# SAP/nested-hashing-psi

Hardware: AMD Instinct MI355X
Metric: server PIE ciphertexts/sec (higher is better)
Workload: dtype u64

## Files before the change

### nested_hashing_psi_amd/csrc/kernels_pie.hip

```cpp
#include <stdlib.h>

#include <cassert>

#include <algorithm>

#include "kernels.hpp"
#include "madasm.h"
#include "stage_a_common.h"
#include "pie_arith.h"

namespace piehip {

static const u32 TPB = 256;

typedef u64 u64x2 __attribute__((ext_vector_type(2)));


template <int BPT>
__global__ void __launch_bounds__(TPB) stage_a_kernel(const DevConsts *__restrict__ dc, u32 N, u32 L, u32 K, u32 b, u32 E,
                                                      const u64 *__restrict__ idx, const u64 *__restrict__ minus,
                                                      const u64 *__restrict__ db, u64 *__restrict__ acc, u32 bstride, u32 h0,
                                                      u32 nq, u32 q)
{
    const u32 n = 2 * (blockIdx.x * TPB + threadIdx.x);
// ... 686 lines not shown
        const Mod qk = ld_mod(c, k);
        u64 col[Lp];
#pragma unroll
        for (u32 j = 0; j < Lp; j++) col[j] = c->tQF_modq[j][k];
        const u64 tp = c->tPinv_modq[k], nq = neg_u(qk.q);
#pragma unroll
        for (int p = 0; p < NP; p++) {
            if (MAD && L <= 6) {
                ColAcc a = {itot[p].lo, 0, 0};
#pragma unroll
                for (u32 j = 0; j < Lp; j++) colacc_mac(a, split30(yp[p][j]), split30(col[j]));
                if (PONLY)
                    ;
                else if (PRE)
                    a.c0 += d[p][k];
                else
                    colacc_mac(a, split30(d[p][k]), split30(tp));
                out[p][k] = (L <= 5 && lz) ? colacc_reduce123_lazy(a, qk, nq) : colacc_reduce<(L > 5)>(a, qk, nq);
            } else {
                U128 acc = dot128<Lp, MAD>(yp[p], col);
                if (PONLY)
                    ;
                else if (PRE)
                    add128(acc, U128{d[p][k], 0});
                else
                    mac128(acc, d[p][k], tp);
                add128(acc, itot[p]);
                out[p][k] = reduce128(acc, qk);
            }
        }
    }
}

template <bool FOLD, u32 L, bool MAD, bool PONLY>
__device__ __forceinline__ void scale_round_comp(const DevConsts *__restrict__ dc, u32 N, u32 n, const u64 *__restrict__ pin,
                                                 u64 *__restrict__ pout, bool fold_out, bool lz)
{
    const u32 H = N / 2;
    constexpr u32 M = 2 * L + 1;
    constexpr int NP = FOLD ? 2 : 1;
    u64 x[NP][M], y[NP][L];
#pragma unroll
    for (u32 a = PONLY ? L : 0; a < M; a++) {
        if (FOLD) {
            PIE_ITER_FENCE();
            const DcC c = dc_iter(dc);
            const u32 ak = a < L ? a : 0, aj = a < L ? 0 : a - L;
            const u64 q = c->mod[a].q, nq = neg_u(q), u = pin[(size_t)a * N], v = pin[(size_t)a * N + H];
            const u64 wa = a < L ? c->fold_iat[ak] : c->fold_iap[aj], was = a < L ? c->fold_iat_sh[ak] : c->fold_iap_sh[aj];
            const u64 wb = a < L ? c->fold_ibt[ak] : c->fold_ibp[aj], wbs = a < L ? c->fold_ibt_sh[ak] : c->fold_ibp_sh[aj];
            x[0][a] = shoup63(u + v, wa, was, nq);
            x[NP - 1][a] = shoup63(u + (4 * q - v), wb, wbs, nq);
        } else {
            x[0][a] = pin[(size_t)a * N];
        }
    }
    scale_round_core<L, MAD, NP, FOLD, PONLY>(dc, x, y, lz);
#pragma unroll
    for (u32 k = 0; k < L; k++) {
        PIE_ITER_FENCE();
        if (FOLD) {
            u64 y0 = y[0][k], y1 = y[NP - 1][k];
            if (fold_out) fold_store(dc, k, y[0][k], y[NP - 1][k], y0, y1);
            pout[(size_t)k * N] = y0;
            pout[(size_t)k * N + H] = y1;
        } else {
            pout[(size_t)k * N] = y[0][k];
        }
    }
}
template <bool FOLD, u32 L, bool MAD, bool P01 = false, bool P2 = false>
__global__ void __launch_bounds__(TPB) scale_round_kernel(const DevConsts *__restrict__ dc, u32 N, const u64 *__restrict__ d,
                                                          u64 *__restrict__ out01, size_t stride01,
                                                          u64 *__restrict__ out2, size_t stride2, u32 fold_comp2)
{
    const u32 n = blockIdx.x * TPB + threadIdx.x;
    if (n >= (FOLD ? N / 2 : N)) return;
    const u32 comp = blockIdx.y, bin = blockIdx.z;
    constexpr u32 M = 2 * L + 1;
    const u64 *pin = d + ((size_t)(bin * 3 + comp) * M) * N + n;
    u64 *pout = comp < 2 ? out01 + (size_t)bin * stride01 + (size_t)comp * L * N + n : out2 + (size_t)bin * stride2 + n;
    const bool lz = FOLD && MAD && comp < 2 && !fold_comp2;
    if (P01 && comp < 2)
        scale_round_comp<FOLD, L, MAD, true>(dc, N, n, pin, pout, true, lz);
    else if (P2 && comp == 2)
        scale_round_comp<FOLD, L, MAD, true>(dc, N, n, pin, pout, fold_comp2, lz);
    else
        scale_round_comp<FOLD, L, MAD, false>(dc, N, n, pin, pout, comp < 2 || fold_comp2, lz);
}
void launch_scale_round(const DevConsts *dc, u32 N, u32 L, const u64 *d, u32 nb, u64 *out01, size_t stride01, u64 *out2,
                        size_t stride2, hipStream_t st, bool small_moduli, bool fold, bool fold_comp2, bool p_only01, bool p_only2)
{
    assert(!p_only01 || (small_moduli && fold_comp2 == p_only2));
    assert(!p_only2 || p_only01);
    dim3 grid(((fold ? N / 2 : N) + TPB - 1) / TPB, 3, nb);
#define SRK2(F_, L_) \
    hipLaunchKernelGGL((scale_round_kernel<F_, L_, true, true, true>), grid, dim3(TPB), 0, st, dc, N, d, out01, stride01, out2, stride2, F_ ? 1u : 0u)
#define SRK(F_, L_, M_, P_) \
    hipLaunchKernelGGL((scale_round_kernel<F_, L_, M_, P_>), grid, dim3(TPB), 0, st, dc, N, d, out01, stride01, out2, stride2, (fold_comp2 && F_) ? 1u : 0u)
#define SRL(L_)                                                                        \
    case L_:                                                                           \
        if (p_only2) {                                                                 \
            if (fold) SRK2(true, L_); else SRK2(false, L_);                            \
        } else if (p_only01) {                                                                \
            if (fold) SRK(true, L_, true, true); else SRK(false, L_, true, true);      \
        } else if (small_moduli) {                                                     \
            if (fold) SRK(true, L_, true, false); else SRK(false, L_, true, false);    \
        } else {                                                                       \
            if (fold) SRK(true, L_, false, false); else SRK(false, L_, false, false);  \
        }                                                                              \
        break;
    switch (L) { SRL(1) SRL(2) SRL(3) SRL(4) SRL(5) SRL(6) SRL(7) }
#undef SRK
#undef SRK2
#undef SRL
}

__device__ __forceinline__ u64 digit_lift(const DevConsts *dc, u32 i, u32 j, u64 v)
{
    const Mod &mj = dc->mod[j];
    const u64 qi = dc->mod[i].q;
    u64 r = (qi < 2 * mj.q) ? (v >= mj.q ? v - mj.q : v) : barrett128(0, v, mj);
    if (v > qi / 2) r = submod(r, dc->qi_modqj[i][j], mj.q);
    return r;
}
template <bool FOLD>
__global__ void __launch_bounds__(TPB) digits_kernel(const DevConsts *__restrict__ dc, u32 N, u32 L, const u64 *__restrict__ d2,
                                                     size_t stride2, u64 *__restrict__ dig)
{
    const u32 n = blockIdx.x * TPB + threadIdx.x;
    const u32 H = N / 2;
    if (n >= (FOLD ? H : N)) return;
    const u32 i = blockIdx.y / L, j = blockIdx.y % L, bin = blockIdx.z;
    const u64 *pin = d2 + (size_t)bin * stride2 + (size_t)i * N + n;
    u64 *pout = dig + (((size_t)bin * L + i) * L + j) * N + n;
    if (FOLD) {
        u64 y0, y1;
        fold_store(dc, j, digit_lift(dc, i, j, pin[0]), digit_lift(dc, i, j, pin[H]), y0, y1);
        pout[0] = y0;
        pout[H] = y1;
    } else {
        pout[0] = digit_lift(dc, i, j, pin[0]);
    }
}
void launch_digits(const DevConsts *dc, u32 N, u32 L, const u64 *d2, size_t stride2, u32 nb, u64 *dig, hipStream_t st, bool fold)
{
    dim3 grid(((fold ? N / 2 : N) + TPB - 1) / TPB, L * L, nb);
    if (fold)
        hipLaunchKernelGGL(digits_kernel<true>, grid, dim3(TPB), 0, st, dc, N, L, d2, stride2, dig);
    else
        hipLaunchKernelGGL(digits_kernel<false>, grid, dim3(TPB), 0, st, dc, N, L, d2, stride2, dig);
}

template <bool MAD, int KP, int RPT = 1, bool EQ = false>
__global__ void __launch_bounds__(TPB) relin_mac_kernel(const DevConsts *__restrict__ dc, u32 N, u32 L, const u64 *__restrict__ d01,
                                                        size_t stride01, const u64 *__restrict__ dig,
                                                        const u64 *__restrict__ key0, const u64 *__restrict__ mask,
                                                        u64 *__restrict__ out, const u32 *__restrict__ out_map,
                                                        size_t key_stride, u32 key_group, u32 T, u32 mask_div, u32 nb,
                                                        const u64 *__restrict__ eqp, u32 eqp_M)
{
    static_assert(RPT == 1 || MAD, "two rows per thread: the column-accumulator path");
    static_assert(!EQ || MAD, "the own-limb term: the column-accumulator path");
    constexpr bool TILE = KP > 0;
    constexpr u32 TT = TILE ? TPB / (KP ? KP : 1) : 1;
    __shared__ u64x2 s_tile[TILE ? 2 * RPT : 1][TILE ? TPB : 1];
    u32 n = 2 * (blockIdx.x * TPB + threadIdx.x);
    u32 std_pair = 0;
    if (TILE) {
        const u32 tiles = T / TT, slice = blockIdx.x / tiles, tau0 = (blockIdx.x % tiles) * TT;
        const u32 k = threadIdx.x / TT, tt = threadIdx.x % TT;
        n = 2 * (slice * KP * T + k * T + tau0 + tt);
        std_pair = slice * KP * T + KP * tau0;
    }
    if (n >= N) return;
    const u32 j = blockIdx.y;
    u32 rows[RPT];
    bool has[RPT];
    if (RPT == 1) {
        rows[0] = blockIdx.z, has[0] = true;
    } else {
        const u32 k = blockIdx.z / key_group, q = blockIdx.z % key_group;
        rows[0] = 2 * k * key_group + q, has[0] = rows[0] < nb;
        rows[RPT - 1] = rows[0] + key_group, has[RPT - 1] = rows[RPT - 1] < nb;
        if (!has[0]) return;
    }
    const u32 bin = rows[0];
    const u64 *key = key0 + (size_t)(bin % key_group) * key_stride;
    const Mod m = dc->mod[j];
    const size_t LN = (size_t)L * N;
    const u32 po = TILE ? 0 : (out_map ? out_map[n] : n);
    u64x2 res[RPT][2];
    if (MAD) {
        ColAcc a[RPT][2][2];
#pragma unroll
        for (int r = 0; r < RPT; r++)
#pragma unroll
            for (int c = 0; c < 2; c++) a[r][c][0] = a[r][c][1] = ColAcc{0, 0, 0};
        for (u32 i = 0; i < L; i++) {
            const u64x2 k0 = *reinterpret_cast<const u64x2 *>(key + (((size_t)i * 2 + 0) * L + j) * N + n);
            const u64x2 k1 = *reinterpret_cast<const u64x2 *>(key + (((size_t)i * 2 + 1) * L + j) * N + n);
            const Split30 k0x = split30(k0.x), k0y = split30(k0.y), k1x = split30(k1.x), k1y = split30(k1.y);
#pragma unroll
            for (int r = 0; r < RPT; r++) {
                if (r && !has[r]) continue;
                const u64x2 d = *reinterpret_cast<const u64x2 *>(dig + (((size_t)rows[r] * L + i) * L + j) * N + n);
                const Split30 dx = split30(d.x), dy = split30(d.y);
                colacc_mac(a[r][0][0], dx, k0x);
                colacc_mac(a[r][0][1], dy, k0y);
                colacc_mac(a[r][1][0], dx, k1x);
                colacc_mac(a[r][1][1], dy, k1y);
            }
        }
        const u64 nq = 0 - m.q;
        if (EQ) {
            const u64 n2q = neg_u(2 * m.q), n4q = neg_u(4 * m.q);
            const u64 tp = dc->tPinv_modq[j], tpsh = dc->tPinv_modq_sh[j];
            const size_t MN = (size_t)eqp_M * N;
#pragma unroll
            for (int r = 0; r < RPT; r++) {
                if (r && !has[r]) continue;
                const u64 *pe = eqp + (size_t)rows[r] * 4 * MN + (size_t)j * N + n;
                const u64x2 va0 = *reinterpret_cast<const u64x2 *>(pe), va1 = *reinterpret_cast<const u64x2 *>(pe + MN),
                            vb0 = *reinterpret_cast<const u64x2 *>(pe + 2 * MN), vb1 = *reinterpret_cast<const u64x2 *>(pe + 3 * MN);
#pragma unroll
                for (int k = 0; k < 2; k++) {
                    const Split30 sa0 = split30(csub_u(csub_u(k ? va0.y : va0.x, n4q), n2q)), sa1 = split30(csub_u(csub_u(k ? va1.y : va1.x, n4q), n2q));
                    const Split30 sb0 = split30(csub_u(csub_u(k ? vb0.y : vb0.x, n4q), n2q)), sb1 = split30(csub_u(csub_u(k ? vb1.y : vb1.x, n4q), n2q));
                    ColAcc t = {0, 0, 0};
                    colacc_mac(t, sa0, sb0);
                    const u64 v0 = shoup63_lazy(colacc_reduce123_lazy(t, m, nq), tp, tpsh, nq);
                    t = ColAcc{0, 0, 0};
                    colacc_mac(t, sa0, sb1);
                    colacc_mac(t, sa1, sb0);
                    const u64 v1 = shoup63_lazy(colacc_reduce123_lazy(t, m, nq), tp, tpsh, nq);
                    a[r][0][k].c0 += v0 & 0x3FFFFFFFull, a[r][0][k].c1 += v0 >> 30;
                    a[r][1][k].c0 += v1 & 0x3FFFFFFFull, a[r][1][k].c1 += v1 >> 30;
                }
            }
        }
#pragma unroll
        for (int r = 0; r < RPT; r++) {
            if (r && !has[r]) continue;
            u64x2 mk;
            if (mask) mk = *reinterpret_cast<const u64x2 *>(mask + (size_t)(rows[r] / mask_div) * LN + (size_t)j * N + n);
#pragma unroll
            for (int c = 0; c < 2; c++) {
                const u64x2 s = *reinterpret_cast<const u64x2 *>(d01 + (size_t)rows[r] * stride01 + (size_t)c * LN + (size_t)j * N + n);
                a[r][c][0].c0 += s.x;
                a[r][c][1].c0 += s.y;
                res[r][c].x = colacc_reduce<false>(a[r][c][0], m, nq);
                res[r][c].y = colacc_reduce<false>(a[r][c][1], m, nq);
                if (mask) {
                    ColAcc p0 = {0, 0, 0}, p1 = {0, 0, 0};
                    colacc_mac(p0, split30(res[r][c].x), split30(mk.x));
                    colacc_mac(p1, split30(res[r][c].y), split30(mk.y));
                    res[r][c].x = colacc_reduce<false>(p0, m, nq);
                    res[r][c].y = colacc_reduce<false>(p1, m, nq);
                }
            }
        }
    } else {
        u64x2 mk;
        if (mask) mk = *reinterpret_cast<const u64x2 *>(mask + (size_t)(bin / mask_div) * LN + (size_t)j * N + n);
        U128 acc[2][2];
#pragma unroll
        for (int c = 0; c < 2; c++)
#pragma unroll
            for (int e = 0; e < 2; e++) acc[c][e] = U128{0, 0};
        for (u32 i = 0; i < L; i++) {
            const u64x2 d = *reinterpret_cast<const u64x2 *>(dig + (((size_t)bin * L + i) * L + j) * N + n);
            const u64x2 k0 = *reinterpret_cast<const u64x2 *>(key + (((size_t)i * 2 + 0) * L + j) * N + n);
            const u64x2 k1 = *reinterpret_cast<const u64x2 *>(key + (((size_t)i * 2 + 1) * L + j) * N + n);
            mac128(acc[0][0], d.x, k0.x);
            mac128(acc[0][1], d.y, k0.y);
            mac128(acc[1][0], d.x, k1.x);
            mac128(acc[1][1], d.y, k1.y);
        }
#pragma unroll
        for (int c = 0; c < 2; c++) {
            const u64x2 s = *reinterpret_cast<const u64x2 *>(d01 + (size_t)bin * stride01 + (size_t)c * LN + (size_t)j * N + n);
            add128(acc[c][0], U128{s.x, 0});
            add128(acc[c][1], U128{s.y, 0});
            res[0][c].x = reduce128(acc[c][0], m);
            res[0][c].y = reduce128(acc[c][1], m);
            if (mask) {
                res[0][c].x = mulmod(res[0][c].x, mk.x, m);
                res[0][c].y = mulmod(res[0][c].y, mk.y, m);
            }
        }
    }
#pragma unroll
    for (int r = 0; r < RPT; r++)
#pragma unroll
        for (int c = 0; c < 2; c++) {
            if (r && !has[r]) continue;
            const u64x2 v = res[r][c];
            if (TILE)
                s_tile[2 * r + c][KP * (threadIdx.x % TT) + threadIdx.x / TT] = v;
            else
                *reinterpret_cast<u64x2 *>(out + ((size_t)rows[r] * 2 + c) * LN + (size_t)j * N + po) = v;
        }
    if (TILE) {
        __syncthreads();
#pragma unroll
        for (int r = 0; r < RPT; r++)
#pragma unroll
            for (int c = 0; c < 2; c++) {
                if (r && !has[r]) continue;
                *reinterpret_cast<u64x2 *>(out + ((size_t)rows[r] * 2 + c) * LN + (size_t)j * N + 2 * (std_pair + threadIdx.x)) = s_tile[2 * r + c][threadIdx.x];
            }
    }
}
void launch_relin_mac(const DevConsts *dc, u32 N, u32 L, const u64 *d01, size_t stride01, const u64 *dig, const u64 *key,
                      const u64 *mask, u64 *out, u32 nb, hipStream_t st, bool small_moduli, const u32 *out_map, size_t key_stride,
                      u32 key_group, u32 sigma_T, u32 sigma_kp, u32 mask_div, const u64 *eqp, u32 eqp_M)
{
    assert(!eqp || (small_moduli && eqp_M >= L));
    if (!key_group) key_group = 1;
    if (!mask_div) mask_div = 1;
    const bool tile = out_map && (sigma_kp == 16 || sigma_kp == 8) && sigma_T >= TPB / sigma_kp && sigma_T % (TPB / sigma_kp) == 0 &&
                      (N / 2) % TPB == 0;
    const int kp = tile ? (int)sigma_kp : 0;
    const bool two = small_moduli && nb >= 2 * key_group;
    const u32 zrows = two ? ((nb + 2 * key_group - 1) / (2 * key_group)) * key_group : nb;
    dim3 grid((N / 2 + TPB - 1) / TPB, L, zrows);
#define RME(M_, K_, R_, E_)                                                                                                            \
    hipLaunchKernelGGL((relin_mac_kernel<M_, K_, R_, E_>), grid, dim3(TPB), 0, st, dc, N, L, d01, stride01, dig, key, mask, out, out_map, \
                       key_stride, key_group, sigma_T, mask_div, nb, eqp, eqp_M)
#define RM(M_, K_, R_) RME(M_, K_, R_, false)
#define RQ(K_, R_) RME(true, K_, R_, true)
    if (eqp && two) {
        if (kp == 16) RQ(16, 2); else if (kp == 8) RQ(8, 2); else RQ(0, 2);
    } else if (eqp) {
        if (kp == 16) RQ(16, 1); else if (kp == 8) RQ(8, 1); else RQ(0, 1);
    } else if (two) {
        if (kp == 16) RM(true, 16, 2); else if (kp == 8) RM(true, 8, 2); else RM(true, 0, 2);
    } else if (small_moduli) {
        if (kp == 16) RM(true, 16, 1); else if (kp == 8) RM(true, 8, 1); else RM(true, 0, 1);
    } else {
        if (kp == 16) RM(false, 16, 1); else if (kp == 8) RM(false, 8, 1); else RM(false, 0, 1);
    }
#undef RQ
#undef RM
#undef RME
}

template <int KP>
__global__ void __launch_bounds__(TPB) deg2_finish_kernel(const DevConsts *__restrict__ dc, u32 N, u32 L, const u64 *__restrict__ d,
                                                          const u64 *__restrict__ eqp, u32 eqp_M, const u64 *__restrict__ mask,
                                                          u64 *__restrict__ out, u32 T, u32 mask_div)
{
    constexpr u32 TT = TPB / KP;
    __shared__ u64x2 s_tile[3][TPB];
    const u32 tiles = T / TT, slice = blockIdx.x / tiles, tau0 = (blockIdx.x % tiles) * TT;
    const u32 kk = threadIdx.x / TT, tt = threadIdx.x % TT;
    const u32 n = 2 * (slice * KP * T + kk * T + tau0 + tt);
    const u32 std_pair = slice * KP * T + KP * tau0;
    const u32 j = blockIdx.y, row = blockIdx.z;
    const Mod m = dc->mod[j];
    const size_t LN = (size_t)L * N, MN = (size_t)eqp_M * N;
    const u64 nq = 0 - m.q, n2q = neg_u(2 * m.q), n4q = neg_u(4 * m.q);
    const u64 tp = dc->tPinv_modq[j], tpsh = dc->tPinv_modq_sh[j];
    const u64 *pe = eqp + (size_t)row * 4 * MN + (size_t)j * N + n;
    const u64x2 va0 = *reinterpret_cast<const u64x2 *>(pe), va1 = *reinterpret_cast<const u64x2 *>(pe + MN),
                vb0 = *reinterpret_cast<const u64x2 *>(pe + 2 * MN), vb1 = *reinterpret_cast<const u64x2 *>(pe + 3 * MN);
    const u64x2 mk = *reinterpret_cast<const u64x2 *>(mask + (size_t)(row / mask_div) * LN + (size_t)j * N + n);
    u64x2 s[3];
#pragma unroll
    for (int c = 0; c < 3; c++) s[c] = *reinterpret_cast<const u64x2 *>(d + ((size_t)row * 3 + c) * LN + (size_t)j * N + n);
    u64 res[3][2];
#pragma unroll
    for (int k = 0; k < 2; k++) {
        const Split30 sa0 = split30(csub_u(csub_u(k ? va0.y : va0.x, n4q), n2q)), sa1 = split30(csub_u(csub_u(k ? va1.y : va1.x, n4q), n2q));
        const Split30 sb0 = split30(csub_u(csub_u(k ? vb0.y : vb0.x, n4q), n2q)), sb1 = split30(csub_u(csub_u(k ? vb1.y : vb1.x, n4q), n2q));
        const Split30 smk = split30(k ? mk.y : mk.x);
        u64 v[3];
        ColAcc t = {0, 0, 0};
        colacc_mac(t, sa0, sb0);
        v[0] = shoup63_lazy(colacc_reduce123_lazy(t, m, nq), tp, tpsh, nq);
        t = ColAcc{0, 0, 0};
        colacc_mac(t, sa0, sb1);
        colacc_mac(t, sa1, sb0);
        v[1] = shoup63_lazy(colacc_reduce123_lazy(t, m, nq), tp, tpsh, nq);
        t = ColAcc{0, 0, 0};
        colacc_mac(t, sa1, sb1);
        v[2] = shoup63_lazy(colacc_reduce123_lazy(t, m, nq), tp, tpsh, nq);
#pragma unroll
        for (int c = 0; c < 3; c++) {
            ColAcc a = {(k ? s[c].y : s[c].x) + (v[c] & 0x3FFFFFFFull), v[c] >> 30, 0};
            ColAcc p = {0, 0, 0};
            colacc_mac(p, split30(colacc_reduce<false>(a, m, nq)), smk);
            res[c][k] = colacc_reduce<false>(p, m, nq);
        }
    }
#pragma unroll
    for (int c = 0; c < 3; c++) s_tile[c][KP * tt + kk] = u64x2{res[c][0], res[c][1]};
    __syncthreads();
#pragma unroll
    for (int c = 0; c < 3; c++)
        *reinterpret_cast<u64x2 *>(out + ((size_t)row * 3 + c) * LN + (size_t)j * N + 2 * (std_pair + threadIdx.x)) = s_tile[c][threadIdx.x];
}
bool deg2_finish_applies(u32 N, u32 sigma_T, u32 sigma_kp)
{
    return sigma_kp == 8 && sigma_T >= TPB / sigma_kp && sigma_T % (TPB / sigma_kp) == 0 && (N / 2) % TPB == 0;
}
void launch_deg2_finish(const DevConsts *dc, u32 N, u32 L, const u64 *d, const u64 *eqp, u32 eqp_M, const u64 *mask, u64 *out, u32 nb,
                        hipStream_t st, u32 sigma_T, u32 sigma_kp, u32 mask_div)
{
    assert(deg2_finish_applies(N, sigma_T, sigma_kp) && eqp_M >= L);
    dim3 grid(N / 2 / TPB, L, nb);
    hipLaunchKernelGGL(deg2_finish_kernel<8>, grid, dim3(TPB), 0, st, dc, N, L, d, eqp, eqp_M, mask, out, sigma_T, mask_div ? mask_div : 1);
}

__global__ void host_flag_kernel(volatile u64 *flag, u64 value)
{
    *flag = value;
    __threadfence_system();
}
void launch_host_flag(u64 *flag_dev, u64 value, hipStream_t st)
{
    hipLaunchKernelGGL(host_flag_kernel, dim3(1), dim3(1), 0, st, (volatile u64 *)flag_dev, value);
}

__global__ void __launch_bounds__(TPB) ct_add_kernel(const DevConsts *dc, u32 N, u32 L, const u64 *__restrict__ x,
                                                     const u64 *__restrict__ y, u64 *__restrict__ out)
{
    const u32 n = blockIdx.x * TPB + threadIdx.x;
    if (n >= N) return;
    const u32 l = blockIdx.y % L;
    const size_t o = ((size_t)blockIdx.z * 2 * L + blockIdx.y) * N + n;
    out[o] = addmod(x[o], y[o], dc->mod[l].q);
}
void launch_ct_add(const DevConsts *dc, u32 N, u32 L, const u64 *x, const u64 *y, u64 *out, u32 nct, hipStream_t st)
{
    dim3 grid((N + TPB - 1) / TPB, 2 * L, nct);
    hipLaunchKernelGGL(ct_add_kernel, grid, dim3(TPB), 0, st, dc, N, L, x, y, out);
}
__global__ void __launch_bounds__(TPB) ct_mul_plain_kernel(const DevConsts *dc, u32 N, u32 L, const u64 *__restrict__ x,
                                                           const u64 *__restrict__ pt, size_t pt_stride,
                                                           u64 *__restrict__ out, u32 pt_div)
{
    const u32 n = blockIdx.x * TPB + threadIdx.x;
    if (n >= N) return;
    const u32 l = blockIdx.y % L;
    const size_t o = ((size_t)blockIdx.z * 2 * L + blockIdx.y) * N + n;
    out[o] = mulmod(x[o], pt[(size_t)(blockIdx.z / pt_div) * pt_stride + (size_t)l * N + n], dc->mod[l]);
}
__global__ void __launch_bounds__(TPB) ctn_mul_plain_kernel(const DevConsts *dc, u32 N, u32 L, const u64 *__restrict__ x,
                                                            const u64 *__restrict__ pt, size_t pt_stride,
                                                            u64 *__restrict__ out, u32 pt_div, u32 comps)
{
    const u32 n = blockIdx.x * TPB + threadIdx.x;
    if (n >= N) return;
    const u32 l = blockIdx.y % L;
    const size_t o = ((size_t)blockIdx.z * comps * L + blockIdx.y) * N + n;
    out[o] = mulmod(x[o], pt[(size_t)(blockIdx.z / pt_div) * pt_stride + (size_t)l * N + n], dc->mod[l]);
}
void launch_ct_mul_plain(const DevConsts *dc, u32 N, u32 L, const u64 *x, const u64 *pt, size_t pt_stride, u64 *out,
                         u32 nct, hipStream_t st, u32 pt_div, u32 comps)
{
    dim3 grid((N + TPB - 1) / TPB, comps * L, nct);
    if (comps == 2)
        hipLaunchKernelGGL(ct_mul_plain_kernel, grid, dim3(TPB), 0, st, dc, N, L, x, pt, pt_stride, out, pt_div ? pt_div : 1);
    else
        hipLaunchKernelGGL(ctn_mul_plain_kernel, grid, dim3(TPB), 0, st, dc, N, L, x, pt, pt_stride, out, pt_div ? pt_div : 1, comps);
}

template <int L, int KEEP>
__global__ void __launch_bounds__(TPB) limb_drop_kernel(const DevConsts *__restrict__ dc, u32 N, u32 blocks_per_poly,
                                                        const u64 *__restrict__ in, u64 *__restrict__ out)
{
    const u32 poly = blockIdx.x / blocks_per_poly;
    const u32 n = (blockIdx.x % blocks_per_poly) * TPB + threadIdx.x;
    if (n >= N) return;
    const u64 *pin = in + (size_t)poly * L * N + n;
    u64 c[L];
#pragma unroll
    for (int i = 0; i < L; i++) c[i] = pin[(size_t)i * N];
#pragma unroll
    for (int l = L - 1; l >= KEEP; l--) {
        const u64 ql = dc->mod[l].q;
        const u64 v = c[l];
        const u64 s = (u64)((int64_t)((ql >> 1) - v) >> 63);
#pragma unroll
        for (int i = 0; i < l; i++) {
            const u64 off = dc->drop_off[l][i];
            const u64 x = c[i] - v + off + (s & (ql - off));
            c[i] = mul_shoup_u(x, dc->drop_inv[l][i], dc->drop_inv_sh[l][i], dc->mod[i].q, dc->drop_negq[i]);
        }
    }
    u64 *pout = out + (size_t)poly * KEEP * N + n;
#pragma unroll
    for (int i = 0; i < KEEP; i++) pout[(size_t)i * N] = c[i];
}
bool launch_limb_drop(const DevConsts *dc, u32 N, u32 L, u32 keep, const u64 *in, u64 *out, u32 npoly, hipStream_t st)
{
    if (keep < 1 || keep >= L || L > MAX_L || !npoly) return false;
    const u32 bpp = (N + TPB - 1) / TPB;
    const dim3 grid(bpp * npoly), block(TPB);
#define DROP_(L_, K_)                                                                                          \
    case (L_) * 8 + (K_):                                                                                      \
        hipLaunchKernelGGL((limb_drop_kernel<L_, K_>), grid, block, 0, st, dc, N, bpp, in, out);               \
        return true
    switch (L * 8 + keep) {
        DROP_(2, 1);
        DROP_(3, 1); DROP_(3, 2);
        DROP_(4, 1); DROP_(4, 2); DROP_(4, 3);
        DROP_(5, 1); DROP_(5, 2); DROP_(5, 3); DROP_(5, 4);
        DROP_(6, 1); DROP_(6, 2); DROP_(6, 3); DROP_(6, 4); DROP_(6, 5);
        DROP_(7, 1); DROP_(7, 2); DROP_(7, 3); DROP_(7, 4); DROP_(7, 5); DROP_(7, 6);
    }
#undef DROP_
    return false;
}

template <u32 L, u32 KEEP, int NP, bool S63>
__device__ __forceinline__ void drop_limbs(const DevConsts *dc, u64 (&c)[NP][L])
{
#pragma unroll
    for (u32 l = L - 1; l >= KEEP; l--) {
        PIE_ITER_FENCE();
        const DcC k = dc_iter(dc);
        const u64 ql = k->mod[l].q;
        u64 v[NP], s[NP];
#pragma unroll
        for (int p = 0; p < NP; p++) {
            v[p] = c[p][l];
            s[p] = (u64)((int64_t)((ql >> 1) - v[p]) >> 63);
        }
#pragma unroll
        for (u32 i = 0; i < l; i++) {
            const u64 off = k->drop_off[l][i], w = k->drop_inv[l][i], wsh = k->drop_inv_sh[l][i], qi = k->mod[i].q;
            const u64 nq = S63 ? neg_u(qi) : k->drop_negq[i];
#pragma unroll
            for (int p = 0; p < NP; p++) {
                const u64 x = c[p][i] - v[p] + off + (s[p] & (ql - off));
                c[p][i] = S63 ? shoup63(x, w, wsh, nq) : mul_shoup_u(x, w, wsh, qi, nq);
            }
        }
    }
}

template <bool FOLD, u32 L, u32 KEEP>
__global__ void __launch_bounds__(TPB) chain_drop_kernel(const DevConsts *__restrict__ dc, u32 N, u32 blocks_per_poly, u64 *data, u32 per,
                                                         size_t gstride)
{
// ... 187 lines not shown
bool launch_expand_both_drop(const DevConsts *dc_parent, const DevConsts *dc_level, u32 N, u32 L, u32 Lc, const u64 *x, size_t sx, size_t six,
                             bool x_drop, const u64 *y, size_t sy, size_t siy, u32 n_outer, u64 *out, hipStream_t st)
{
    if (!expand_both_drop_applies(L, Lc)) return false;
    dim3 grid((N / 2 + TPB - 1) / TPB, n_outer * 4);
#define EBD_(L_, C_)                                                                                                                     \
    if (L == L_ && Lc == C_) {                                                                                                           \
        if (x_drop)                                                                                                                      \
            hipLaunchKernelGGL((expand_both_drop_kernel<L_, C_, true>), grid, dim3(TPB), 0, st, dc_parent, dc_level, N, x, sx, six, y, sy, siy, out, n_outer);  \
        else                                                                                                                             \
            hipLaunchKernelGGL((expand_both_drop_kernel<L_, C_, false>), grid, dim3(TPB), 0, st, dc_parent, dc_level, N, x, sx, six, y, sy, siy, out, n_outer); \
        return true;                                                                                                                     \
    }
    PIE_CHAIN_DROP_PAIRS(EBD_)
#undef EBD_
    return false;
}
bool launch_expand_both_drop_xy(const DevConsts *dc_parent, const DevConsts *dc_x, const DevConsts *dc_level, u32 N, u32 L, u32 Lx, u32 Lc,
                                const u64 *x, size_t sx, size_t six, const u64 *y, size_t sy, size_t siy, u32 n_outer, u64 *out, hipStream_t st)
{
    if (Lx == L) return launch_expand_both_drop(dc_parent, dc_level, N, L, Lc, x, sx, six, true, y, sy, siy, n_outer, out, st);
    if (!expand_both_drop_xy_applies(L, Lx, Lc)) return false;
    dim3 grid((N / 2 + TPB - 1) / TPB, n_outer * 4);
#define EBX_(L_, X_, C_)                                                                                                                  \
    if (L == L_ && Lx == X_ && Lc == C_) {                                                                                               \
        hipLaunchKernelGGL((expand_both_drop_xy_kernel<L_, X_, C_>), grid, dim3(TPB), 0, st, dc_parent, dc_x, dc_level, N, x, sx, six, y, sy, \
                           siy, out, n_outer);                                                                                           \
        return true;                                                                                                                     \
    }
    PIE_CHAIN_DROP_TRIPLES(EBX_)
#undef EBX_
    return false;
}

__global__ void __launch_bounds__(TPB) permute_kernel(u32 N, const u64 *__restrict__ in, const u32 *__restrict__ map,
                                                      u64 *__restrict__ out)
{
    const u32 p = blockIdx.x * TPB + threadIdx.x;
    if (p >= N) return;
    const size_t r = (size_t)blockIdx.y * N;
    out[r + p] = in[r + map[p]];
}
void launch_permute(u32 N, const u64 *in, const u32 *map, u64 *out, u32 nrows, hipStream_t st)
{
    dim3 grid((N + TPB - 1) / TPB, nrows);
    hipLaunchKernelGGL(permute_kernel, grid, dim3(TPB), 0, st, N, in, map, out);
}

__global__ void __launch_bounds__(TPB) bcast_mul_plain_kernel(const DevConsts *dc, u32 N, u32 L, const u64 *__restrict__ x,
                                                              size_t xs, u32 group, const u64 *__restrict__ pt, size_t ps_outer,
                                                              size_t ps_inner, u64 *__restrict__ out)
{
    const u32 n = blockIdx.x * TPB + threadIdx.x;
    if (n >= N) return;
    const u32 l = blockIdx.y % L, i = blockIdx.z, g = i / group, r = i % group;
    const size_t LN = (size_t)L * N;
    const size_t o = (size_t)blockIdx.y * N + n;
    out[(size_t)i * 2 * LN + o] = mulmod(x[(size_t)g * xs + o], pt[(size_t)g * ps_outer + (size_t)r * ps_inner + (size_t)l * N + n], dc->mod[l]);
}
void launch_bcast_mul_plain(const DevConsts *dc, u32 N, u32 L, const u64 *x, size_t xs, u32 group, const u64 *pt, size_t ps_outer,
                            size_t ps_inner, u64 *out, u32 nct, hipStream_t st)
{
    dim3 grid((N + TPB - 1) / TPB, 2 * L, nct);
    hipLaunchKernelGGL(bcast_mul_plain_kernel, grid, dim3(TPB), 0, st, dc, N, L, x, xs, group, pt, ps_outer, ps_inner, out);
}
__global__ void __launch_bounds__(TPB) rot_prepare_kernel(const DevConsts *dc, u32 N, u32 L, const u64 *__restrict__ x,
                                                          const u32 *__restrict__ maps, u32 map_group, u32 acc, u32 identity_first,
                                                          u64 *__restrict__ d01, u64 *__restrict__ d2)
{
    const u32 p = blockIdx.x * TPB + threadIdx.x;
    if (p >= N) return;
    const u32 l = blockIdx.y, i = blockIdx.z, r = i % map_group;
    const size_t LN = (size_t)L * N;
    const u64 *c0 = x + (size_t)i * 2 * LN + (size_t)l * N, *c1 = c0 + LN;
    u64 *o0 = d01 + (size_t)i * 2 * LN + (size_t)l * N, *o1 = o0 + LN, *o2 = d2 + (size_t)i * LN + (size_t)l * N;
    if (identity_first && r == 0) {
        o0[p] = c0[p];
        o1[p] = c1[p];
        o2[p] = 0;
        return;
    }
    const u32 s = maps[(size_t)r * N + p];
    const u64 q = dc->mod[l].q;
    o0[p] = acc ? addmod(c0[p], c0[s], q) : c0[s];
    o1[p] = acc ? c1[p] : 0;
    o2[p] = c1[s];
}
void launch_rot_prepare(const DevConsts *dc, u32 N, u32 L, const u64 *x, const u32 *maps, u32 map_group, bool acc, bool identity_first,
                        u64 *d01, u64 *d2, u32 nct, hipStream_t st)
{
    dim3 grid((N + TPB - 1) / TPB, L, nct);
    hipLaunchKernelGGL(rot_prepare_kernel, grid, dim3(TPB), 0, st, dc, N, L, x, maps, map_group ? map_group : 1u, acc ? 1u : 0u,
                       identity_first ? 1u : 0u, d01, d2);
}
__global__ void __launch_bounds__(TPB) sum_mul_plain_kernel(const DevConsts *dc, u32 N, u32 L, const u64 *__restrict__ x, u32 group,
                                                            const u64 *__restrict__ pt, size_t pt_stride, u64 *__restrict__ out,
                                                            size_t out_stride)
{
    const u32 n = blockIdx.x * TPB + threadIdx.x;
    if (n >= N) return;
    const u32 l = blockIdx.y % L, g = blockIdx.z;
    const size_t LN = (size_t)L * N;
    const size_t o = (size_t)blockIdx.y * N + n;
    const Mod m = dc->mod[l];
    u64 s = 0;
    for (u32 r = 0; r < group; r++) s = addmod(s, x[((size_t)g * group + r) * 2 * LN + o], m.q);
    out[(size_t)g * out_stride + o] = mulmod(s, pt[(size_t)g * pt_stride + (size_t)l * N + n], m);
}
void launch_sum_mul_plain(const DevConsts *dc, u32 N, u32 L, const u64 *x, u32 group, const u64 *pt, size_t pt_stride, u64 *out,
                          size_t out_stride, u32 ngroups, hipStream_t st)
{
    dim3 grid((N + TPB - 1) / TPB, 2 * L, ngroups);
    hipLaunchKernelGGL(sum_mul_plain_kernel, grid, dim3(TPB), 0, st, dc, N, L, x, group, pt, pt_stride, out, out_stride);
}

__global__ void __launch_bounds__(TPB) encode_scatter_kernel(const DevConsts *dc, u32 N, u32 M,
                                                             const int64_t *__restrict__ slots, u32 B,
                                                             const u32 *__restrict__ inv_pos, u64 *__restrict__ u)
{
    const u32 p = blockIdx.x * TPB + threadIdx.x;
    if (p >= N) return;
    const u64 t = dc->mod[M].q;
    const u32 s = inv_pos[p];
    u64 val = 0;
    if (s < B) {
        const int64_t v = slots[(size_t)blockIdx.y * B + s];
        const u64 mag = v < 0 ? (u64)(-v) : (u64)v;
        val = v < 0 ? (mag ? t - mag : 0) : mag;
    }
    u[(size_t)blockIdx.y * N + p] = val;
}
void launch_encode_scatter(const DevConsts *dc, u32 N, u32 M, const int64_t *slots, u32 B, const u32 *inv_pos, u64 *u,
                           u32 npt, hipStream_t st)
{
    dim3 grid((N + TPB - 1) / TPB, npt);
    hipLaunchKernelGGL(encode_scatter_kernel, grid, dim3(TPB), 0, st, dc, N, M, slots, B, inv_pos, u);
}
__global__ void __launch_bounds__(TPB) encode_lift_kernel(const DevConsts *dc, u32 N, u32 L, u32 M,
                                                          const u64 *__restrict__ u, u64 *__restrict__ out, u32 l0)
{
    const u32 n = blockIdx.x * TPB + threadIdx.x;
    if (n >= N) return;
    const u64 t = dc->mod[M].q;
    const u64 v = u[(size_t)blockIdx.z * N + n];
    const u64 q = dc->mod[l0 + blockIdx.y].q;
    out[((size_t)blockIdx.z * L + blockIdx.y) * N + n] = v > t / 2 ? q - (t - v) : v;
}
void launch_encode_lift(const DevConsts *dc, u32 N, u32 L, u32 M, const u64 *u, u64 *out, u32 npt, hipStream_t st, u32 l0)
{
    dim3 grid((N + TPB - 1) / TPB, L, npt);
    hipLaunchKernelGGL(encode_lift_kernel, grid, dim3(TPB), 0, st, dc, N, L, M, u, out, l0);
}

}
```

Before: 78270.

## Merge own-limb tensor products into relin accumulator columns before a single reduction

Adds a merged relinearization kernel for small L that feeds the own-limb tensor products (a0*b0, a0*b1+a1*b0) straight into the column accumulators alongside the key-digit products. This replaces the separate lazy reduction and Shoup multiply per product. It pre-multiplies b by tPinv with a Shoup step so a single final reduction suffices. The deg2 finish kernel gets the same change. The aim is fewer modular reductions per coefficient, at the cost of a new kernel variant and tighter accumulator-headroom bounds guarded by static asserts.

```diff
diff --git a/nested_hashing_psi_amd/csrc/kernels_pie.hip b/nested_hashing_psi_amd/csrc/kernels_pie.hip
--- a/nested_hashing_psi_amd/csrc/kernels_pie.hip
+++ b/nested_hashing_psi_amd/csrc/kernels_pie.hip
@@ -862,6 +862,25 @@
         hipLaunchKernelGGL(digits_kernel<false>, grid, dim3(TPB), 0, st, dc, N, L, d2, stride2, dig);
 }
 
+#ifndef PIEHIP_RELIN_EQ_MERGED
+#define PIEHIP_RELIN_EQ_MERGED 1
+#endif
+static const u32 RELIN_EQ_MERGED_MAX_L = 6;
+static_assert(RELIN_EQ_MERGED_MAX_L + 2 <= COLACC_MAX_TERMS, "column 1 takes two products below 2^60 per term: 16 of them at the most");
+static_assert(((u64)(RELIN_EQ_MERGED_MAX_L + 2) << 60) <= (1ull << 63), "column 0 holds d01 < 2^63 beside the products");
+struct OwnLimbOps {
+    Split30 a0, a1, b0, b1;
+};
+__device__ __forceinline__ OwnLimbOps own_limb_ops(u64 a0, u64 a1, u64 b0, u64 b1, u64 tp, u64 tpsh, u64 nq, u64 n2q, u64 n4q)
+{
+    OwnLimbOps o;
+    o.a0 = split30(csub_u(csub_u(csub_u(a0, n4q), n2q), nq));
+    o.a1 = split30(csub_u(csub_u(csub_u(a1, n4q), n2q), nq));
+    o.b0 = split30(shoup63(b0, tp, tpsh, nq));
+    o.b1 = split30(shoup63(b1, tp, tpsh, nq));
+    return o;
+}
+
 template <bool MAD, int KP, int RPT = 1, bool EQ = false>
 __global__ void __launch_bounds__(TPB) relin_mac_kernel(const DevConsts *__restrict__ dc, u32 N, u32 L, const u64 *__restrict__ d01,
                                                         size_t stride01, const u64 *__restrict__ dig,
@@ -1022,6 +1041,11 @@
             }
     }
 }
+#if PIEHIP_RELIN_EQ_MERGED
+static void launch_relin_mac_merged(dim3 grid, int kp, bool two, const DevConsts *dc, u32 N, u32 L, const u64 *d01, size_t stride01,
+                                    const u64 *dig, const u64 *key, const u64 *mask, u64 *out, u32 nb, hipStream_t st, const u32 *out_map,
+                                    size_t key_stride, u32 key_group, u32 sigma_T, u32 mask_div, const u64 *eqp, u32 eqp_M);
+#endif
 void launch_relin_mac(const DevConsts *dc, u32 N, u32 L, const u64 *d01, size_t stride01, const u64 *dig, const u64 *key,
                       const u64 *mask, u64 *out, u32 nb, hipStream_t st, bool small_moduli, const u32 *out_map, size_t key_stride,
                       u32 key_group, u32 sigma_T, u32 sigma_kp, u32 mask_div, const u64 *eqp, u32 eqp_M)
@@ -1035,6 +1059,13 @@
     const bool two = small_moduli && nb >= 2 * key_group;
     const u32 zrows = two ? ((nb + 2 * key_group - 1) / (2 * key_group)) * key_group : nb;
     dim3 grid((N / 2 + TPB - 1) / TPB, L, zrows);
+#if PIEHIP_RELIN_EQ_MERGED
+    if (eqp && L <= RELIN_EQ_MERGED_MAX_L) {
+        launch_relin_mac_merged(grid, kp, two, dc, N, L, d01, stride01, dig, key, mask, out, nb, st, out_map, key_stride, key_group, sigma_T,
+                                mask_div, eqp, eqp_M);
+        return;
+    }
+#endif
 #define RME(M_, K_, R_, E_)                                                                                                            \
     hipLaunchKernelGGL((relin_mac_kernel<M_, K_, R_, E_>), grid, dim3(TPB), 0, st, dc, N, L, d01, stride01, dig, key, mask, out, out_map, \
                        key_stride, key_group, sigma_T, mask_div, nb, eqp, eqp_M)
@@ -1082,6 +1113,23 @@
     u64 res[3][2];
 #pragma unroll
     for (int k = 0; k < 2; k++) {
+#if PIEHIP_RELIN_EQ_MERGED
+        const OwnLimbOps o = own_limb_ops(k ? va0.y : va0.x, k ? va1.y : va1.x, k ? vb0.y : vb0.x, k ? vb1.y : vb1.x, tp, tpsh, nq, n2q, n4q);
+        const Split30 smk = split30(k ? mk.y : mk.x);
+        ColAcc a[3];
+#pragma unroll
+        for (int c = 0; c < 3; c++) a[c] = ColAcc{k ? s[c].y : s[c].x, 0, 0};
+        colacc_mac(a[0], o.a0, o.b0);
+        colacc_mac(a[1], o.a0, o.b1);
+        colacc_mac(a[1], o.a1, o.b0);
+        colacc_mac(a[2], o.a1, o.b1);
+#pragma unroll
+        for (int c = 0; c < 3; c++) {
+            ColAcc p = {0, 0, 0};
+            colacc_mac(p, split30(colacc_reduce123_lazy(a[c], m, nq)), smk);
+            res[c][k] = colacc_reduce<false>(p, m, nq);
+        }
+#else
         const Split30 sa0 = split30(csub_u(csub_u(k ? va0.y : va0.x, n4q), n2q)), sa1 = split30(csub_u(csub_u(k ? va1.y : va1.x, n4q), n2q));
         const Split30 sb0 = split30(csub_u(csub_u(k ? vb0.y : vb0.x, n4q), n2q)), sb1 = split30(csub_u(csub_u(k ? vb1.y : vb1.x, n4q), n2q));
         const Split30 smk = split30(k ? mk.y : mk.x);
@@ -1103,6 +1151,7 @@
             colacc_mac(p, split30(colacc_reduce<false>(a, m, nq)), smk);
             res[c][k] = colacc_reduce<false>(p, m, nq);
         }
+#endif
     }
 #pragma unroll
     for (int c = 0; c < 3; c++) s_tile[c][KP * tt + kk] = u64x2{res[c][0], res[c][1]};
@@ -1596,4 +1645,141 @@
     hipLaunchKernelGGL(encode_lift_kernel, grid, dim3(TPB), 0, st, dc, N, L, M, u, out, l0);
 }
 
-}
+#if PIEHIP_RELIN_EQ_MERGED
+template <int KP, int RPT>
+__global__ void __launch_bounds__(TPB) relin_mac_merged_kernel(const DevConsts *__restrict__ dc, u32 N, u32 L, const u64 *__restrict__ d01,
+                                                               size_t stride01, const u64 *__restrict__ dig,
+                                                               const u64 *__restrict__ key0, const u64 *__restrict__ mask,
+                                                               u64 *__restrict__ out, const u32 *__restrict__ out_map,
+                                                               size_t key_stride, u32 key_group, u32 T, u32 mask_div, u32 nb,
+                                                               const u64 *__restrict__ eqp, u32 eqp_M)
+{
+    constexpr bool TILE = KP > 0;
+    constexpr u32 TT = TILE ? TPB / (KP ? KP : 1) : 1;
+    __shared__ u64x2 s_tile[TILE ? 2 * RPT : 1][TILE ? TPB : 1];
+    u32 n = 2 * (blockIdx.x * TPB + threadIdx.x);
+    u32 std_pair = 0;
+    if (TILE) {
+        const u32 tiles = T / TT, slice = blockIdx.x / tiles, tau0 = (blockIdx.x % tiles) * TT;
+        const u32 k = threadIdx.x / TT, tt = threadIdx.x % TT;
+        n = 2 * (slice * KP * T + k * T + tau0 + tt);
+        std_pair = slice * KP * T + KP * tau0;
+    }
+    if (n >= N) return;
+    const u32 j = blockIdx.y;
+    u32 rows[RPT];
+    bool has[RPT];
+    if (RPT == 1) {
+        rows[0] = blockIdx.z, has[0] = true;
+    } else {
+        const u32 k = blockIdx.z / key_group, q = blockIdx.z % key_group;
+        rows[0] = 2 * k * key_group + q, has[0] = rows[0] < nb;
+        rows[RPT - 1] = rows[0] + key_group, has[RPT - 1] = rows[RPT - 1] < nb;
+        if (!has[0]) return;
+    }
+    const u64 *key = key0 + (size_t)(rows[0] % key_group) * key_stride;
+    const Mod m = dc->mod[j];
+    const size_t LN = (size_t)L * N, MN = (size_t)eqp_M * N;
+    const u32 po = TILE ? 0 : (out_map ? out_map[n] : n);
+    const u64 nq = 0 - m.q, n2q = neg_u(2 * m.q), n4q = neg_u(4 * m.q);
+    const u64 tp = dc->tPinv_modq[j], tpsh = dc->tPinv_modq_sh[j];
+    ColAcc a[RPT][2][2];
+    u64x2 e[RPT][4], mk[RPT];
+#pragma unroll
+    for (int r = 0; r < RPT; r++) {
+        if (r && !has[r]) continue;
+#pragma unroll
+        for (int c = 0; c < 2; c++) {
+            const u64x2 s = *reinterpret_cast<const u64x2 *>(d01 + (size_t)rows[r] * stride01 + (size_t)c * LN + (size_t)j * N + n);
+            a[r][c][0] = ColAcc{s.x, 0, 0};
+            a[r][c][1] = ColAcc{s.y, 0, 0};
+        }
+        const u64 *pe = eqp + (size_t)rows[r] * 4 * MN + (size_t)j * N + n;
+#pragma unroll
+        for (int s = 0; s < 4; s++) e[r][s] = *reinterpret_cast<const u64x2 *>(pe + s * MN);
+        if (mask) mk[r] = *reinterpret_cast<const u64x2 *>(mask + (size_t)(rows[r] / mask_div) * LN + (size_t)j * N + n);
+    }
+#pragma unroll
+    for (int r = 0; r < RPT; r++) {
+        if (r && !has[r]) continue;
+#pragma unroll
+        for (int k = 0; k < 2; k++) {
+            const OwnLimbOps o = own_limb_ops(k ? e[r][0].y : e[r][0].x, k ? e[r][1].y : e[r][1].x, k ? e[r][2].y : e[r][2].x,
+                                              k ? e[r][3].y : e[r][3].x, tp, tpsh, nq, n2q, n4q);
+            colacc_mac(a[r][0][k], o.a0, o.b0);
+            colacc_mac(a[r][1][k], o.a0, o.b1);
+            colacc_mac(a[r][1][k], o.a1, o.b0);
+        }
+    }
+    for (u32 i = 0; i < L; i++) {
+        const u64x2 k0 = *reinterpret_cast<const u64x2 *>(key + (((size_t)i * 2 + 0) * L + j) * N + n);
+        const u64x2 k1 = *reinterpret_cast<const u64x2 *>(key + (((size_t)i * 2 + 1) * L + j) * N + n);
+        const Split30 k0x = split30(k0.x), k0y = split30(k0.y), k1x = split30(k1.x), k1y = split30(k1.y);
+#pragma unroll
+        for (int r = 0; r < RPT; r++) {
+            if (r && !has[r]) continue;
+            const u64x2 d = *reinterpret_cast<const u64x2 *>(dig + (((size_t)rows[r] * L + i) * L + j) * N + n);
+            const Split30 dx = split30(d.x), dy = split30(d.y);
+            colacc_mac(a[r][0][0], dx, k0x);
+            colacc_mac(a[r][0][1], dy, k0y);
+            colacc_mac(a[r][1][0], dx, k1x);
+            colacc_mac(a[r][1][1], dy, k1y);
+        }
+    }
+    u64x2 res[RPT][2];
+#pragma unroll
+    for (int r = 0; r < RPT; r++) {
+        if (r && !has[r]) continue;
+#pragma unroll
+        for (int c = 0; c < 2; c++) {
+            if (mask) {
+                ColAcc p0 = {0, 0, 0}, p1 = {0, 0, 0};
+                colacc_mac(p0, split30(colacc_reduce123_lazy(a[r][c][0], m, nq)), split30(mk[r].x));
+                colacc_mac(p1, split30(colacc_reduce123_lazy(a[r][c][1], m, nq)), split30(mk[r].y));
+                res[r][c].x = colacc_reduce<false>(p0, m, nq);
+                res[r][c].y = colacc_reduce<false>(p1, m, nq);
+            } else {
+                res[r][c].x = colacc_reduce<false>(a[r][c][0], m, nq);
+                res[r][c].y = colacc_reduce<false>(a[r][c][1], m, nq);
+            }
+        }
+    }
+#pragma unroll
+    for (int r = 0; r < RPT; r++)
+#pragma unroll
+        for (int c = 0; c < 2; c++) {
+            if (r && !has[r]) continue;
+            if (TILE)
+                s_tile[2 * r + c][KP * (threadIdx.x % TT) + threadIdx.x / TT] = res[r][c];
+            else
+                *reinterpret_cast<u64x2 *>(out + ((size_t)rows[r] * 2 + c) * LN + (size_t)j * N + po) = res[r][c];
+        }
+    if (TILE) {
+        __syncthreads();
+#pragma unroll
+        for (int r = 0; r < RPT; r++)
+#pragma unroll
+            for (int c = 0; c < 2; c++) {
+                if (r && !has[r]) continue;
+                *reinterpret_cast<u64x2 *>(out + ((size_t)rows[r] * 2 + c) * LN + (size_t)j * N + 2 * (std_pair + threadIdx.x)) = s_tile[2 * r + c][threadIdx.x];
+            }
+    }
+}
+static void launch_relin_mac_merged(dim3 grid, int kp, bool two, const DevConsts *dc, u32 N, u32 L, const u64 *d01, size_t stride01,
+                                    const u64 *dig, const u64 *key, const u64 *mask, u64 *out, u32 nb, hipStream_t st, const u32 *out_map,
+                                    size_t key_stride, u32 key_group, u32 sigma_T, u32 mask_div, const u64 *eqp, u32 eqp_M)
+{
+    assert(L <= RELIN_EQ_MERGED_MAX_L && eqp);
+#define RG(K_, R_)                                                                                                                        \
+    hipLaunchKernelGGL((relin_mac_merged_kernel<K_, R_>), grid, dim3(TPB), 0, st, dc, N, L, d01, stride01, dig, key, mask, out, out_map, \
+                       key_stride, key_group, sigma_T, mask_div, nb, eqp, eqp_M)
+    if (two) {
+        if (kp == 16) RG(16, 2); else if (kp == 8) RG(8, 2); else RG(0, 2);
+    } else {
+        if (kp == 16) RG(16, 1); else if (kp == 8) RG(8, 1); else RG(0, 1);
+    }
+#undef RG
+}
+#endif
+
+}
```

Result: no change. 79040 (median of 6 runs) (+1.0%).
